# Jiang-Muyun/PointNet12

Hardware: AMD Instinct MI355X
Metric: points/sec fwd+bwd, PointNet2 SemSeg B=16x4096 pts (higher is better)
Workload: dtype f32 (wide-layer products: exact bf16x3 operand splits, 6 bf16 MFMAs per fp32 product, fp32 accumulate)

## Files before the change

### pointnet12_amd/csrc/mlp_res.hip

```cpp
#include "mlp_host.h"
#include "split_bf16.h"

namespace {

constexpr int RES_BM = 64;

struct ResPlan {
    signed char dx_rb[8], dx_cj[8];
    signed char dw_cj[8], dw_q0[8], dw_q1[8];
};

inline bool make_res_plan(int CI_T, ResPlan *out) {
    ResPlan p;
    int load[8], next_q[4] = {0, 0, 0, 0};
    for (int w = 0; w < 8; ++w) { p.dx_rb[w] = p.dx_cj[w] = -1; p.dw_cj[w] = 0; p.dw_q0[w] = p.dw_q1[w] = 0; load[w] = 0; }
    if (CI_T < 1 || CI_T > 4) return false;
    for (int i = 0; i < 2 * CI_T; ++i) { p.dx_rb[i] = (signed char)(i & 1); p.dx_cj[i] = (signed char)(i >> 1); load[i] = 2; }
    const int target = CI_T > 2 ? CI_T : 2;
    for (int pass = 0; pass < 2; ++pass)
        for (int w = 7; w >= 0; --w) {
            if ((pass == 0) != (p.dx_rb[w] < 0) || p.dw_q0[w] != p.dw_q1[w]) continue;
            int cj = -1;
            for (int c = 0; c < CI_T; ++c)
                if (next_q[c] < 4 && (cj < 0 || next_q[c] < next_q[cj])) cj = c;
// ... 612 lines not shown
                            frags(e0, pb, f0);
                            if (two) {
                                frags(e1, pb, f1);
#pragma unroll
                                for (int q = 0; q < 6; ++q) {
                                    accw[DXW ? 0 : j] = __builtin_amdgcn_mfma_f32_32x32x16_bf16(f0[PA[q]].v, f0[PB[q]].v, accw[DXW ? 0 : j], 0, 0, 0);
                                    accw[DXW || j + 1 >= TW ? 0 : j + 1] = __builtin_amdgcn_mfma_f32_32x32x16_bf16(f1[PA[q]].v, f1[PB[q]].v, accw[DXW || j + 1 >= TW ? 0 : j + 1], 0, 0, 0);
                                }
                            } else {
#pragma unroll
                                for (int q = 0; q < 6; ++q)
                                    accw[DXW ? 0 : j] = __builtin_amdgcn_mfma_f32_32x32x16_bf16(f0[PA[q]].v, f0[PB[q]].v, accw[DXW ? 0 : j], 0, 0, 0);
                            }
                        }
                    }
                }
                RSTAMP(3)
            } else {
                f32x16 acc, acc2;
#pragma unroll
                for (int r = 0; r < 16; ++r) { acc[r] = 0.f; acc2[r] = 0.f; }
#pragma unroll
                for (int kb = 0; kb < KBX; ++kb) {
                    const unsigned o = tr_img_off(l31, 2 * kb + lh);
                    SplitFrag ah, am, al;
                    ah.q = *reinterpret_cast<const uint4 *>(ia + o);
                    am.q = *reinterpret_cast<const uint4 *>(ia + o + PANEL);
                    al.q = *reinterpret_cast<const uint4 *>(ia + o + 2 * PANEL);
                    acc = __builtin_amdgcn_mfma_f32_32x32x16_bf16(al.v, wh[DXW ? kb : 0].v, acc, 0, 0, 0);
                    f32x16 &d = DX2 ? acc2 : acc;
                    SplitFrag wlo;
                    if (WL_LDS) wlo.q = wl_lds[kb * 64]; else wlo = wl[DXW && !WL_LDS ? kb : 0];
                    d = __builtin_amdgcn_mfma_f32_32x32x16_bf16(ah.v, wlo.v, d, 0, 0, 0);
                    acc = __builtin_amdgcn_mfma_f32_32x32x16_bf16(am.v, wm[DXW ? kb : 0].v, acc, 0, 0, 0);
                    d = __builtin_amdgcn_mfma_f32_32x32x16_bf16(am.v, wh[DXW ? kb : 0].v, d, 0, 0, 0);
                    acc = __builtin_amdgcn_mfma_f32_32x32x16_bf16(ah.v, wm[DXW ? kb : 0].v, acc, 0, 0, 0);
                    d = __builtin_amdgcn_mfma_f32_32x32x16_bf16(ah.v, wh[DXW ? kb : 0].v, d, 0, 0, 0);
                }
#ifdef PN2_STAMP
                { float a0_ = acc[0] + acc2[0]; asm volatile("" : "+v"(a0_)); }
#endif
                RSTAMP(3)
                const float *yq = Yps + buf * (BP * LDP) + (4 * lh) * LDP + ecol;
                float yv[16];
                if (MASKED) {
#pragma unroll
                    for (int r = 0; r < 16; ++r) yv[r] = yq[((r & 3) + 8 * (r >> 2)) * LDP];
                }
                float *xb = dX + ((size_t)chunk * BP + 4 * lh) * (unsigned)ldxo;
                unsigned offx = (unsigned)ecol;
                asm volatile("" : "+v"(offx));
                float s0 = 0.f, s1 = 0.f;
                const float *x0q = x0s + buf * (BP * 12) + (4 * lh) * 12;
                const unsigned sgn = (unsigned)(chunk & 1) << 31;
#pragma unroll
                for (int r = 0; r < 16; ++r) {
                    float dz = __uint_as_float(__float_as_uint(DX2 ? acc[r] + acc2[r] : acc[r]) ^ sgn);
                    if (MASKED) {
                        const float y = yv[r];
                        dz = bn_act(y, emu, esc, ebe) > 0.f ? dz : 0.f;
                        s0 += dz;
                        s1 = __builtin_fmaf(dz, (y - emu) * eis, s1);
                    }
                    if (FUSE0) {
                        const float4 *xr = reinterpret_cast<const float4 *>(x0q + ((r & 3) + 8 * (r >> 2)) * 12);
                        const float4 a0 = xr[0], a1 = xr[1], a2 = xr[2];
                        g0[0] = __builtin_fmaf(dz, a0.x, g0[0]); g0[FUSE0 ? 1 : 0] = __builtin_fmaf(dz, a0.y, g0[FUSE0 ? 1 : 0]);
                        g0[FUSE0 ? 2 : 0] = __builtin_fmaf(dz, a0.z, g0[FUSE0 ? 2 : 0]); g0[FUSE0 ? 3 : 0] = __builtin_fmaf(dz, a0.w, g0[FUSE0 ? 3 : 0]);
                        g0[FUSE0 ? 4 : 0] = __builtin_fmaf(dz, a1.x, g0[FUSE0 ? 4 : 0]); g0[FUSE0 ? 5 : 0] = __builtin_fmaf(dz, a1.y, g0[FUSE0 ? 5 : 0]);
                        g0[FUSE0 ? 6 : 0] = __builtin_fmaf(dz, a1.z, g0[FUSE0 ? 6 : 0]); g0[FUSE0 ? 7 : 0] = __builtin_fmaf(dz, a1.w, g0[FUSE0 ? 7 : 0]);
                        g0[FUSE0 ? 8 : 0] = __builtin_fmaf(dz, a2.x, g0[FUSE0 ? 8 : 0]); g0[FUSE0 ? 9 : 0] = __builtin_fmaf(dz, a2.y, g0[FUSE0 ? 9 : 0]);
                        g0[FUSE0 ? 10 : 0] = __builtin_fmaf(dz, a2.z, g0[FUSE0 ? 10 : 0]); g0[FUSE0 ? 11 : 0] = __builtin_fmaf(dz, a2.w, g0[FUSE0 ? 11 : 0]);
                    } else {
#if defined(PN2_EXP_NOSTORE)
                        if (dz == 1.2345e-33f) xb[offx] = dz;
#elif defined(PN2_EXP_PLAINSTORE)
                        xb[offx] = dz;
#else
                        PN2_STREAM_STORE(dz, xb + offx);
#endif
                    }
                    offx += ((r & 3) == 3 ? 5u : 1u) * (unsigned)ldxo;
                }
                if (MASKED) { st0 += (double)s0; st1 += (double)s1; }
                RSTAMP(4)
            }
            chunk += G;
            buf ^= 1;
        };
        while (chunk < chunks) {
            iter(D2 ? raw1 : raw0);
            if (chunk >= chunks) break;
            iter(raw0);
        }
        RSTAMP_FLUSH(wave)
        RABS(wave, 2)
        if (!DXW) {
#pragma unroll
            for (int j = 0; j < TW; ++j) {
                const int e = (wave - CI_T) + j * NDW;
                if (e < NTILE) {
                    const int mb = e / CI_T, nb = e - mb * CI_T;
#pragma unroll
                    for (int r = 0; r < 16; ++r)
                        atomicAdd(dW + (int64_t)(mb * 32 + acc_row(r, lh)) * lddw + nb * 32 + l31, accw[DXW ? 0 : j][r]);
                }
            }
        } else if (MASKED && red_p != nullptr) {
            st0 += __shfl_xor(st0, 32, 64);
            st1 += __shfl_xor(st1, 32, 64);
            if (lh == 0) {
                double *rep = red_p + (size_t)(blockIdx.x % PN2_STAT_REPLICAS) * 2 * Ci;
                atomicAdd(rep + ecol, st0);
                atomicAdd(rep + Ci + ecol, st1);
            }
        }
        if (DXW && FUSE0) {
#pragma unroll
            for (int j = 0; j < (DXW && FUSE0 ? 12 : 1); ++j) g0[j] += __shfl_xor(g0[j], 32, 64);
            if (lh == 0) {
                float *pr = part0 + ((size_t)(blockIdx.x % PN2_CF_REPL) * Ci + ecol) * 16;
#pragma unroll
                for (int j = 0; j < (DXW && FUSE0 ? 12 : 1); ++j) atomicAdd(pr + j, g0[j]);
            }
        }
    };
    if (has_dx) run(pn2_true{}); else run(pn2_false{});
    RABS(wave, 3)
}

template <int CO_T, int CI_T, bool POOLED, bool MASKED, bool FUSE0 = false>
int launch_split_bwd_res(ResDy dy, const float *Yp, int ldp, const float *aff_p, const float *W, int ldw, int64_t tiles, float *dX, int ldxo,
                         double *red_p, float *dW, int lddw, hipStream_t s, const float *X0 = nullptr, int ld0 = 0, float *part0 = nullptr) {
    constexpr int Co = 32 * CO_T, Ci = 32 * CI_T;
    constexpr size_t lds = 2 * 6 * (size_t)(32 * 256) + sizeof(float) * (2 * 32 * (Ci + 4) + 8 * Co + 6 * Ci + (FUSE0 ? 2 * 32 * 12 : 0)) +
                           (CO_T == 4 && CI_T < 4 ? (size_t)CI_T * (Co / 16) * 1024 : 0);
    static_assert(lds <= 160 * 1024, "LDS");
    if (!aligned16(dy.Y) || !aligned16(Yp)) return PN2_EUNSUPPORTED;
    auto kern = split_bwd_res_kernel<CO_T, CI_T, POOLED, MASKED, FUSE0>;
    static Pn2PerDevice raised;
    if (pn2_raise_dynamic_lds(reinterpret_cast<const void *>(kern), raised) != PN2_OK) return PN2_ELAUNCH;
    const int64_t chunks = tiles * (RES_BM / 32), cap = pn2_num_cus();
    PN2_NOTE_KERNEL(kern);
    hipLaunchKernelGGL(kern, dim3((unsigned)(chunks < cap ? chunks : cap)), dim3(512), lds, s, dy, Yp, ldp, aff_p, W, ldw, chunks, dX, ldxo,
                       red_p, dW, lddw, X0, ld0, part0);
    return pn2_launch_status();
}

template <int CO_T, int CI_T>
__global__ __launch_bounds__(512, 1) void split_bwd_cf_kernel(const float *dZp, const int32_t *arg, int ldo, int kshift, const float *W2 ,
                                                              const float *Yp, int ldp, const float *aff_p, int64_t chunks, float *dX, int ldxo, double *red_p,
                                                              float *slab) {
    constexpr int Co = 32 * CO_T, Ci = 32 * CI_T, BP = 32, QD = Co / 4, QP = Ci / 4, LDP = Ci + 4;
    constexpr int PANEL = BP * 256, BUF = 6 * PANEL;
    constexpr int KBX = Co / 16, KBM = Ci / 16, KBT = KBX + KBM;
    constexpr int NS = 8 - CI_T - 1, NTS = 64 * NS;
    constexpr int NGT = CI_T * (CI_T + 1) / 2, LDT = Co + Ci + 4;
    static_assert(NS >= CO_T, "one staging wave per D column");
    constexpr int RPP = NTS / QD, IT_D = (BP + RPP - 1) / RPP, IT_P = (BP * QP + NTS - 1) / NTS;
    static_assert(NTS % QD == 0, "one channel quad of D per staging thread");
    unsigned char *lds_b = reinterpret_cast<unsigned char *>(res_lds);
    float *Yps = res_lds + (2 * BUF) / 4;
    float *xtab = Yps + 2 * BP * LDP;
    const int t = threadIdx.x, lane = t & 63, wave = __builtin_amdgcn_readfirstlane(t >> 6), l31 = lane & 31, lh = lane >> 5;
    const int G = gridDim.x;
    RABS(wave, 0)
    for (int i = t; i < 3 * Ci; i += 512) { const float v = aff_p[i]; xtab[i] = v; xtab[3 * Ci + i] = i < Ci ? v : -v; }

    const bool has_dx = wave < CI_T, is_gram = wave == CI_T;
    const int ecol = (has_dx ? wave : 0) * 32 + l31;
    const int ts = wave <= CI_T ? 0 : t - 64 * (CI_T + 1);
    struct Raw { float4 z; int4 a; float4 p[IT_P]; };
    Raw raw;
    auto p_item = [&](int i, int &row, int &q) { const int idx = (NTS * (i + 1) > BP * QP) ? min(ts + NTS * i, BP * QP - 1) : ts + NTS * i; row = idx / QP; q = idx - row * QP; };
    auto fetch = [&](int64_t chunk) {
        const unsigned m0 = (unsigned)(chunk < chunks ? chunk : chunks - 1) * BP;
        const unsigned o = (m0 >> kshift) * (unsigned)ldo + 4u * (unsigned)(ts % QD);
        raw.z = ld4(dZp + o);
        raw.a = ld4i(arg + o);
#pragma unroll
        for (int i = 0; i < IT_P; ++i) {
            int row, q;
            p_item(i, row, q);
            raw.p[i] = ld4(Yp + ((m0 + (unsigned)row) * (unsigned)ldp + 4u * (unsigned)q));
        }
    };
    auto store_split = [&](unsigned char *img, int row, int q, const float4 v) {
        unsigned h0, m0, l0, h1, m1, l1;
        split2(v.x, v.y, h0, m0, l0);
        split2(v.z, v.w, h1, m1, l1);
        const unsigned o = tr_img_off(row, q >> 1) + 8u * (unsigned)(q & 1);
        *reinterpret_cast<uint2 *>(img + o) = make_uint2(h0, h1);
        *reinterpret_cast<uint2 *>(img + o + PANEL) = make_uint2(m0, m1);
        *reinterpret_cast<uint2 *>(img + o + 2 * PANEL) = make_uint2(l0, l1);
    };
    auto stage = [&](int64_t chunk, int buf) {
        unsigned char *ia = lds_b + buf * BUF, *ib = ia + 3 * PANEL;
        float *yp = Yps + buf * (BP * LDP);
        const unsigned m0 = (unsigned)(chunk < chunks ? chunk : chunks - 1) * BP;
        const int kbase = (int)(m0 & ((1u << kshift) - 1u));
        const int par = (int)(chunk & 1);
        const float *xt = xtab + par * (3 * Ci);
        const float lim = par ? -INFINITY : INFINITY;
        {
            unsigned h0, m0_, l0, h1, m1, l1;
            split2(raw.z.x, raw.z.y, h0, m0_, l0);
            split2(raw.z.z, raw.z.w, h1, m1, l1);
            const unsigned sm2 = par ? 0x80008000u : 0u;
            h0 ^= sm2; m0_ ^= sm2; l0 ^= sm2; h1 ^= sm2; m1 ^= sm2; l1 ^= sm2;
            const int q = ts % QD, r0 = ts / QD;
            const int4 a = raw.a;
#pragma unroll
            for (int i = 0; i < IT_D; ++i) {
                const int row = (RPP * (i + 1) > BP) ? min(r0 + RPP * i, BP - 1) : r0 + RPP * i;
                const int k = kbase + row;
                const unsigned k0 = (a.x == k ? 0x0000ffffu : 0u) | (a.y == k ? 0xffff0000u : 0u);
                const unsigned k1 = (a.z == k ? 0x0000ffffu : 0u) | (a.w == k ? 0xffff0000u : 0u);
                const unsigned o = tr_img_off(row, q >> 1) + 8u * (unsigned)(q & 1);
                *reinterpret_cast<uint2 *>(ia + o) = make_uint2(h0 & k0, h1 & k1);
                *reinterpret_cast<uint2 *>(ia + o + PANEL) = make_uint2(m0_ & k0, m1 & k1);
                *reinterpret_cast<uint2 *>(ia + o + 2 * PANEL) = make_uint2(l0 & k0, l1 & k1);
            }
        }
#pragma unroll
        for (int i = 0; i < IT_P; ++i) {
            int row, q;
            p_item(i, row, q);
            float4 x = raw.p[i];
            *reinterpret_cast<float4 *>(&yp[row * LDP + 4 * q]) = x;
            const float4 mu = *reinterpret_cast<const float4 *>(&xt[4 * q]), sc = *reinterpret_cast<const float4 *>(&xt[Ci + 4 * q]);
            const float4 be = *reinterpret_cast<const float4 *>(&xt[2 * Ci + 4 * q]);
            x.x = __builtin_amdgcn_fmed3f(bn_act(x.x, mu.x, sc.x, be.x), 0.f, lim); x.y = __builtin_amdgcn_fmed3f(bn_act(x.y, mu.y, sc.y, be.y), 0.f, lim);
            x.z = __builtin_amdgcn_fmed3f(bn_act(x.z, mu.z, sc.z, be.z), 0.f, lim); x.w = __builtin_amdgcn_fmed3f(bn_act(x.w, mu.w, sc.w, be.w), 0.f, lim);
            store_split(ib, row, q, x);
        }
    };
    auto raw_landed = [&]() {
        asm volatile("" : "+v"(raw.z.x), "+v"(raw.z.y), "+v"(raw.z.z), "+v"(raw.z.w));
        asm volatile("" : "+v"(raw.a.x), "+v"(raw.a.y), "+v"(raw.a.z), "+v"(raw.a.w));
#pragma unroll
        for (int i = 0; i < IT_P; ++i) asm volatile("" : "+v"(raw.p[i].x), "+v"(raw.p[i].y), "+v"(raw.p[i].z), "+v"(raw.p[i].w));
    };
    const int g16 = lane >> 4, j16 = lane & 15, tq = j16 >> 2, tp = j16 & 3;
    auto frag_t = [&](const unsigned char *img, int cblk, int pb) {
        const int c0 = (cblk * 32 + 16 * (g16 & 1)) >> 3;
        SplitFrag f;
#pragma unroll
        for (int r2 = 0; r2 < 2; ++r2) {
            const int row = 16 * pb + 8 * (g16 >> 1) + 4 * r2 + tq;
            const unsigned o = tr_img_off(row, c0 + (tp >> 1)) + 8u * (unsigned)(tp & 1);
            const pn2_s16x4 v = __builtin_amdgcn_ds_read_tr16_b64_v4i16(
                reinterpret_cast<__attribute__((address_space(3))) pn2_s16x4 *>((__attribute__((address_space(3))) unsigned char *)(img) + o));
            const uint2 u = __builtin_bit_cast(uint2, v);
            f.u[2 * r2] = u.x; f.u[2 * r2 + 1] = u.y;
        }
        return f;
    };

    if (has_dx) {
        SplitFrag wh[KBT], wm[KBT], wl[KBM];
        uint4 *wl_lds = reinterpret_cast<uint4 *>(xtab + 6 * Ci) + (size_t)wave * KBX * 64 + lane;
        {
            float v[KBT][8];
#pragma unroll
            for (int kb = 0; kb < KBT; ++kb)
#pragma unroll
                for (int e = 0; e < 8; ++e) v[kb][e] = W2[(16 * kb + 8 * lh + e) * Ci + ecol];
#pragma unroll
            for (int kb = 0; kb < KBT; ++kb) {
                SplitFrag lo;
#pragma unroll
                for (int e = 0; e < 4; ++e) split2(v[kb][2 * e], v[kb][2 * e + 1], wh[kb].u[e], wm[kb].u[e], lo.u[e]);
                if (kb < KBX) wl_lds[kb * 64] = lo.q; else wl[kb < KBX ? 0 : kb - KBX] = lo;
            }
        }
        Affine a(aff_p, Ci);
        const float emu = a.mean[ecol], esc = a.scale[ecol], ebe = a.beta[ecol], eis = a.invstd[ecol];
        const float eh = W2[(Co + Ci) * Ci + ecol];
        double st0 = 0.0, st1 = 0.0, st2 = 0.0;
        int64_t chunk = blockIdx.x;
        int buf = 0;
        __syncthreads();
        RABS(wave, 1)
        RSTAMP_DECL
        while (chunk < chunks) {
            __syncthreads();
            RSTAMP(2)
            const unsigned char *ia = lds_b + buf * BUF, *ib = ia + 3 * PANEL;
            f32x16 acc, acc2;
#pragma unroll
            for (int r = 0; r < 16; ++r) { acc[r] = 0.f; acc2[r] = 0.f; }
#ifndef PN2_X_CF_NODXM
#pragma unroll
            for (int kb = 0; kb < KBT; ++kb) {
                const unsigned char *img = kb < KBX ? ia : ib;
                const unsigned o = tr_img_off(l31, 2 * (kb < KBX ? kb : kb - KBX) + lh);
                SplitFrag ah, am, al, wlo;
                ah.q = *reinterpret_cast<const uint4 *>(img + o);
                am.q = *reinterpret_cast<const uint4 *>(img + o + PANEL);
                al.q = *reinterpret_cast<const uint4 *>(img + o + 2 * PANEL);
                if (kb < KBX) wlo.q = wl_lds[kb * 64]; else wlo = wl[kb < KBX ? 0 : kb - KBX];
                acc = __builtin_amdgcn_mfma_f32_32x32x16_bf16(al.v, wh[kb].v, acc, 0, 0, 0);
                acc2 = __builtin_amdgcn_mfma_f32_32x32x16_bf16(ah.v, wlo.v, acc2, 0, 0, 0);
                acc = __builtin_amdgcn_mfma_f32_32x32x16_bf16(am.v, wm[kb].v, acc, 0, 0, 0);
                acc2 = __builtin_amdgcn_mfma_f32_32x32x16_bf16(am.v, wh[kb].v, acc2, 0, 0, 0);
                acc = __builtin_amdgcn_mfma_f32_32x32x16_bf16(ah.v, wm[kb].v, acc, 0, 0, 0);
                acc2 = __builtin_amdgcn_mfma_f32_32x32x16_bf16(ah.v, wh[kb].v, acc2, 0, 0, 0);
            }
#endif
#ifdef PN2_STAMP
            { float a0_ = acc[0] + acc2[0]; asm volatile("" : "+v"(a0_)); }
#endif
            RSTAMP(3)
#ifdef PN2_X_CF_NOEPI
            if (acc[0] == 1.2345e-33f) dX[0] = acc2[1];
            chunk += G; buf ^= 1;
            continue;
#endif
            const float *yq = Yps + buf * (BP * LDP) + (4 * lh) * LDP + ecol;
            float yv[16];
#pragma unroll
            for (int r = 0; r < 16; ++r) yv[r] = yq[((r & 3) + 8 * (r >> 2)) * LDP];
            float *xb = dX + ((size_t)chunk * BP + 4 * lh) * (unsigned)ldxo;
            unsigned offx = (unsigned)ecol;
            asm volatile("" : "+v"(offx));
            float s0 = 0.f, s1 = 0.f, s2 = 0.f;
            const unsigned sgn = (unsigned)(chunk & 1) << 31;
#pragma unroll
            for (int r = 0; r < 16; ++r) {
                const float y = yv[r];
                const float x = bn_act(y, emu, esc, ebe);
                float dz = __uint_as_float(__float_as_uint(acc[r] + acc2[r]) ^ sgn) + eh;
                dz = x > 0.f ? dz : 0.f;
                s0 += dz;
                s1 = __builtin_fmaf(dz, (y - emu) * eis, s1);
                s2 += fmaxf(x, 0.f);
                PN2_STREAM_STORE(dz, xb + offx);
                offx += ((r & 3) == 3 ? 5u : 1u) * (unsigned)ldxo;
            }
            st0 += (double)s0; st1 += (double)s1; st2 += (double)s2;
            RSTAMP(4)
            chunk += G;
            buf ^= 1;
        }
        RSTAMP_FLUSH(wave)
        RABS(wave, 2)
        st0 += __shfl_xor(st0, 32, 64);
        st1 += __shfl_xor(st1, 32, 64);
        st2 += __shfl_xor(st2, 32, 64);
        if (lh == 0) {
            if (red_p != nullptr) {
                double *rep = red_p + (size_t)(blockIdx.x % PN2_STAT_REPLICAS) * 2 * Ci;
                atomicAdd(rep + ecol, st0);
                atomicAdd(rep + Ci + ecol, st1);
            }
            slab[(size_t)blockIdx.x * (Ci * LDT) + (size_t)ecol * LDT + Co + Ci] = (float)st2;
        }
    } else {
        constexpr int PA[6] = {2, 0, 1, 1, 0, 0}, PB[6] = {0, 2, 1, 0, 1, 0};
        auto mm2 = [&](f32x16 &c0, const SplitFrag (&a0)[3], const SplitFrag (&b0)[3], f32x16 &c1, const SplitFrag (&a1)[3], const SplitFrag (&b1)[3]) {
#pragma unroll
            for (int q = 0; q < 6; ++q) {
                c0 = __builtin_amdgcn_mfma_f32_32x32x16_bf16(a0[PA[q]].v, b0[PB[q]].v, c0, 0, 0, 0);
                c1 = __builtin_amdgcn_mfma_f32_32x32x16_bf16(a1[PA[q]].v, b1[PB[q]].v, c1, 0, 0, 0);
            }
        };
        auto mm1 = [&](f32x16 &c0, const SplitFrag (&a0)[3], const SplitFrag (&b0)[3]) {
#pragma unroll
            for (int q = 0; q < 6; ++q) c0 = __builtin_amdgcn_mfma_f32_32x32x16_bf16(a0[PA[q]].v, b0[PB[q]].v, c0, 0, 0, 0);
        };
        auto frag3 = [&](const unsigned char *img, int blk, int pb, SplitFrag (&f)[3]) {
            f[0] = frag_t(img, blk, pb); f[1] = frag_t(img + PANEL, blk, pb); f[2] = frag_t(img + 2 * PANEL, blk, pb);
        };
        float *sl = slab + (size_t)blockIdx.x * (Ci * LDT);
        if (is_gram) {
            f32x16 accg[NGT];
#pragma unroll
            for (int j = 0; j < NGT; ++j)
#pragma unroll
                for (int r = 0; r < 16; ++r) accg[j][r] = 0.f;
            int64_t chunk = blockIdx.x;
            int buf = 0;
            __syncthreads();
            RABS(wave, 1)
            RSTAMP_DECL
            while (chunk < chunks) {
                __syncthreads();
                RSTAMP(2)
#ifndef PN2_X_CF_NOT
                const unsigned char *ib = lds_b + buf * BUF + 3 * PANEL;
#pragma unroll
                for (int pb = 0; pb < BP / 16; ++pb) {
                    SplitFrag fx[CI_T][3];
#pragma unroll
                    for (int i = 0; i < CI_T; ++i) frag3(ib, i, pb, fx[i]);
                    if constexpr (CI_T == 1) {
                        mm1(accg[0], fx[0], fx[0]);
                    } else if constexpr (CI_T == 2) {
                        mm2(accg[0], fx[0], fx[0], accg[1], fx[0], fx[1]);
                        mm1(accg[2], fx[1], fx[1]);
                    } else {
                        static_assert(CI_T <= 3, "Gram tiles");
                        mm2(accg[0], fx[0], fx[0], accg[1], fx[0], fx[1]);
                        mm2(accg[2], fx[1], fx[1], accg[3], fx[0], fx[2]);
                        mm2(accg[4], fx[1], fx[2], accg[5], fx[2], fx[2]);
                    }
                }
#endif
                RSTAMP(3)
                chunk += G;
                buf ^= 1;
            }
            RSTAMP_FLUSH(wave)
            RABS(wave, 2)
#pragma unroll
            for (int j = 0; j < CI_T; ++j)
#pragma unroll
                for (int i = 0; i <= j; ++i) {
                    const f32x16 &acc = accg[j * (j + 1) / 2 + i];
#pragma unroll
                    for (int r = 0; r < 16; ++r) sl[(i * 32 + acc_row(r, lh)) * LDT + Co + j * 32 + l31] = acc[r];
                    if (i != j) {
#pragma unroll
                        for (int r = 0; r < 16; ++r) sl[(j * 32 + l31) * LDT + Co + i * 32 + acc_row(r, lh)] = acc[r];
                    }
                }
        } else {
            f32x16 accw[CI_T];
#pragma unroll
            for (int j = 0; j < CI_T; ++j)
#pragma unroll
                for (int r = 0; r < 16; ++r) accw[j][r] = 0.f;
            const int nb = wave - CI_T - 1 < CO_T ? wave - CI_T - 1 : -1;
            int64_t chunk = blockIdx.x;
            fetch(chunk);
            __syncthreads();
            stage(chunk, 0);
            fetch(chunk + G);
            raw_landed();
            int buf = 0;
            RABS(wave, 1)
            RSTAMP_DECL
            while (chunk < chunks) {
                __syncthreads();
                RSTAMP(2)
#ifndef PN2_X_CF_NOSTAGE
                stage(chunk + G, buf ^ 1);
#endif
                RSTAMP(0)
#ifndef PN2_X_CF_NOFETCH
                fetch(chunk + 2 * (int64_t)G);
#endif
                __builtin_amdgcn_sched_barrier(0);
                RSTAMP(1)
#ifndef PN2_X_CF_NOT
                if (nb >= 0) {
                    const unsigned char *ia = lds_b + buf * BUF, *ib = ia + 3 * PANEL;
#pragma unroll
                    for (int pb = 0; pb < BP / 16; ++pb) {
                        SplitFrag fb[3], fa0[3], fa1[3];
                        frag3(ia, nb, pb, fb);
                        frag3(ib, 0, pb, fa0);
                        if constexpr (CI_T >= 2) {
                            frag3(ib, 1, pb, fa1);
                            mm2(accw[0], fa0, fb, accw[CI_T >= 2 ? 1 : 0], fa1, fb);
                            if constexpr (CI_T == 3) {
                                frag3(ib, 2, pb, fa0);
                                mm1(accw[CI_T == 3 ? 2 : 0], fa0, fb);
                            }
                        } else {
                            mm1(accw[0], fa0, fb);
                        }
                    }
                }
#endif
                RSTAMP(3)
                chunk += G;
                buf ^= 1;
            }
            RSTAMP_FLUSH(wave)
            RABS(wave, 2)
            if (nb >= 0) {
#pragma unroll
                for (int i = 0; i < CI_T; ++i)
#pragma unroll
                    for (int r = 0; r < 16; ++r) sl[(i * 32 + acc_row(r, lh)) * LDT + nb * 32 + l31] = accw[i][r];
            }
        }
    }
    RABS(wave, 3)
}

__global__ __launch_bounds__(128) void cf_prep_kernel(LazyCoef lc, const float *coef, int ldc, const float *__restrict__ W, int ldw,
                                                      const float *__restrict__ bias, int Co, int Ci, float *__restrict__ W2) {
    __shared__ double fac[256];
    lazy_coef_prologue(lc);
    const float *c0 = coef, *q1 = coef + ldc, *q0 = coef + 2 * ldc, *mean = coef + 3 * ldc;
    const int r = blockIdx.x;
    if (r < Co) {
        for (int i = threadIdx.x; i < Ci; i += 128) W2[r * Ci + i] = c0[r] * W[(int64_t)r * ldw + i];
        return;
    }
    const int j = r - Co;
    for (int c = threadIdx.x; c < Co; c += 128)
        fac[c] = j == Ci ? ((double)q1[c] * ((double)bias[c] - (double)mean[c]) + (double)q0[c]) : (double)W[(int64_t)c * ldw + j] * (double)q1[c];
    __syncthreads();
    for (int i = threadIdx.x; i < Ci; i += 128) {
        double s0 = 0.0, s1 = 0.0, s2 = 0.0, s3 = 0.0;
#pragma unroll 4
        for (int c = 0; c < Co; c += 4) {
            s0 += fac[c] * (double)W[(int64_t)c * ldw + i];
            s1 += fac[c + 1] * (double)W[(int64_t)(c + 1) * ldw + i];
            s2 += fac[c + 2] * (double)W[(int64_t)(c + 2) * ldw + i];
            s3 += fac[c + 3] * (double)W[(int64_t)(c + 3) * ldw + i];
        }
        W2[r * Ci + i] = (float)((s0 + s1) + (s2 + s3));
    }
}

__global__ __launch_bounds__(256) void cf_finish_kernel(const float *__restrict__ slab, int nslab, int Co, int Ci, const float *coef, int ldc,
                                                        const float *__restrict__ W, int ldw, const float *__restrict__ bias,
                                                        float *__restrict__ dW, int lddw) {
    extern __shared__ double cf_row[];
    const int i = blockIdx.x, LDT = Co + Ci + 4, NQ = LDT / 4;
    const int q = threadIdx.x & 63, sg = threadIdx.x >> 6;
    double a0 = 0.0, a1 = 0.0, a2 = 0.0, a3 = 0.0;
    if (q < NQ) {
        const float *p = slab + (size_t)i * LDT + 4 * q;
        const size_t ss = (size_t)Ci * LDT;
        int w = sg;
        for (; w + 28 < nslab; w += 32) {
            float4 v[8];
#pragma unroll
            for (int e = 0; e < 8; ++e) v[e] = ld4(p + (size_t)(w + 4 * e) * ss);
#pragma unroll
            for (int e = 0; e < 8; ++e) { a0 += (double)v[e].x; a1 += (double)v[e].y; a2 += (double)v[e].z; a3 += (double)v[e].w; }
        }
        for (; w < nslab; w += 4) {
            const float4 v = ld4(p + (size_t)w * ss);
            a0 += (double)v.x; a1 += (double)v.y; a2 += (double)v.z; a3 += (double)v.w;
        }
        double *d = cf_row + sg * LDT + 4 * q;
        d[0] = a0; d[1] = a1; d[2] = a2; d[3] = a3;
    }
    __syncthreads();
    for (int n = threadIdx.x; n < LDT; n += 256) cf_row[n] = (cf_row[n] + cf_row[LDT + n]) + (cf_row[2 * LDT + n] + cf_row[3 * LDT + n]);
    __syncthreads();
    const float *c0 = coef, *q1 = coef + ldc, *q0 = coef + 2 * ldc, *mean = coef + 3 * ldc;
    const double sx = cf_row[Co + Ci];
    for (int c = threadIdx.x; c < Co; c += 256) {
        double dot = 0.0;
        for (int j = 0; j < Ci; ++j) dot += (double)W[(int64_t)c * ldw + j] * cf_row[Co + j];
        const double g = (double)c0[c] * cf_row[c] + (double)q1[c] * (dot + ((double)bias[c] - (double)mean[c]) * sx) + (double)q0[c] * sx;
        dW[(int64_t)c * lddw + i] += (float)g;
    }
}

template <int CO_T, int CI_T>
int launch_split_bwd_cf(const float *dZp, const int32_t *arg, int ldo, int kshift, const float *coef, LazyCoef lc, const float *W, int ldw,
                        const float *bias, const float *Yp, int ldp, const float *aff_p, int64_t P, float *dX, int ldxo, double *red_p,
                        float *dW, int lddw, float *scratch, hipStream_t s) {
    constexpr int Co = 32 * CO_T, Ci = 32 * CI_T, LDT = Co + Ci + 4;
    constexpr size_t lds = 2 * 6 * (size_t)(32 * 256) + sizeof(float) * (2 * 32 * (Ci + 4) + 6 * Ci) + (size_t)CI_T * (Co / 16) * 1024;
    static_assert(lds <= 160 * 1024, "LDS");
    auto kern = split_bwd_cf_kernel<CO_T, CI_T>;
    static Pn2PerDevice raised;
    if (pn2_raise_dynamic_lds(reinterpret_cast<const void *>(kern), raised) != PN2_OK) return PN2_ELAUNCH;
    float *W2 = scratch, *slab = scratch + (((Co + Ci + 1) * Ci + 63) & ~63);
    const int64_t chunks = P / 32, cap = pn2_num_cus() < 256 ? pn2_num_cus() : 256;
    const int grid = (int)(chunks < cap ? chunks : cap);
    hipLaunchKernelGGL(cf_prep_kernel, dim3(Co + Ci + 1), dim3(128), 0, s, lc, coef, round4(Co), W, ldw, bias, Co, Ci, W2);
    PN2_NOTE_KERNEL(kern);
    hipLaunchKernelGGL(kern, dim3((unsigned)grid), dim3(512), lds, s, dZp, arg, ldo, kshift, W2, Yp, ldp, aff_p, chunks, dX, ldxo, red_p, slab);
    hipLaunchKernelGGL(cf_finish_kernel, dim3(Ci), dim3(256), sizeof(double) * 4 * LDT, s, slab, grid, Co, Ci, coef, round4(Co), W, ldw, bias,
                       dW, lddw);
    return pn2_launch_status();
}

#define PN2_RES_CASE(CO, CI, POOL, MASKED)                                                                                \
    if (Co == CO && Ci == CI)                                                                                              \
        return launch_bwd_res<CO / 32, CI / 32, POOL, MASKED>(dy, Yp, ldp, aff_p, W, ldw, tiles, dX, ldxo, red_p, dW, lddw, s);

int dispatch_bwd_res(int Kpool, bool masked, int Co, int Ci, ResDy dy, const float *Yp, int ldp, const float *aff_p, const float *W,
                     int ldw, int64_t tiles, float *dX, int ldxo, double *red_p, float *dW, int lddw, hipStream_t s) {
    if (pn2_opt(PN2_OPT_SPLIT) && pn2_opt(PN2_OPT_SPLIT_RES)) {
#define PN2_SPLIT_RES_CASE(CO, CI, POOLED, MASKED)                                                                        \
        if (Co == CO && Ci == CI) {                                                                                        \
            const int rc = launch_split_bwd_res<CO / 32, CI / 32, POOLED, MASKED>(dy, Yp, ldp, aff_p, W, ldw, tiles, dX, ldxo, red_p, dW, lddw, s); \
            if (rc != PN2_EUNSUPPORTED) return rc;                                                                         \
        }
        const bool all = pn2_opt(PN2_OPT_SPLIT_RES) >= 2;
        if (Kpool == 0 && masked) {
            if (all) { PN2_SPLIT_RES_CASE(32, 32, false, true) }
            PN2_SPLIT_RES_CASE(64, 64, false, true) PN2_SPLIT_RES_CASE(96, 64, false, true)
            if (tiles >= pn2_opt(PN2_OPT_SPLIT_RES_MIN_TILES_128)) { PN2_SPLIT_RES_CASE(128, 128, false, true) }
        } else if (Kpool == 0) {
            if (tiles >= pn2_opt(PN2_OPT_SPLIT_RES_MIN_TILES_128)) { PN2_SPLIT_RES_CASE(128, 128, false, false) }
        } else if (masked && Kpool % 32 == 0) {
            if (all) { PN2_SPLIT_RES_CASE(64, 32, true, true) }
            PN2_SPLIT_RES_CASE(128, 64, true, true) PN2_SPLIT_RES_CASE(128, 96, true, true)
        }
#undef PN2_SPLIT_RES_CASE
    }
    if (Kpool == 0 && masked) {
        PN2_RES_CASE(32, 32, 0, true) PN2_RES_CASE(64, 64, 0, true) PN2_RES_CASE(96, 64, 0, true)
        if (tiles >= 4096) { PN2_RES_CASE(128, 128, 0, true) }
    } else if (Kpool == 0) {
        if (tiles >= 4096) { PN2_RES_CASE(128, 128, 0, false) }
    } else if (masked && Kpool % 64 == 0) {
        PN2_RES_CASE(128, 64, 1, true) PN2_RES_CASE(128, 96, 1, true)
    } else if (masked && Kpool == 32) {
        PN2_RES_CASE(64, 32, 2, true) PN2_RES_CASE(128, 64, 2, true)
    }
    return PN2_EUNSUPPORTED;
}

struct ResPool {
    float2 *rec;
    const float *gamma;
    int ldp, U;
    LazyBn lz;
};

template <int K_T, int N_T, bool ACT, int POOL>
__global__ __launch_bounds__(512, 2) void fwd_res_kernel(const float *__restrict__ X, int ldx, const float *aff ,
                                                         const float *__restrict__ W, int ldw, const float *__restrict__ bias,
                                                         float *__restrict__ Y, int ldy, int64_t slabs, double *__restrict__ stats,
                                                         ResPool pool) {
    constexpr int K = 32 * K_T, N = 32 * N_T, LDA = K + 4, QK = K / 4, IT = 32 * QK / 64;
    const int NW = blockDim.x >> 6;
    float *Ws = res_lds;
    float *atab = Ws + N * LDA;
    const int t = threadIdx.x, lane = t & 63, wave = __builtin_amdgcn_readfirstlane(t >> 6), l31 = lane & 31, lh = lane >> 5;
    float *Ab = atab + 3 * K + wave * (32 * LDA);
    RABS(wave, 0)

    lazy_bn_prologue(pool.lz);
    for (int i = t; i < N * QK; i += blockDim.x) {
        const int n = i / QK, q = i - n * QK;
        const float *src = W + (int64_t)n * ldw + 4 * q;
        float4 v;
        if ((ldw & 3) == 0 && (reinterpret_cast<uintptr_t>(W) & 15) == 0) v = ld4(src);
        else v = make_float4(src[0], src[1], src[2], src[3]);
        *reinterpret_cast<float4 *>(&Ws[n * LDA + 4 * q]) = v;
    }
    if (ACT)
        for (int i = t; i < 3 * K; i += blockDim.x) atab[i] = aff[i];
    float bj[N_T];
#pragma unroll
    for (int j = 0; j < N_T; ++j) bj[j] = bias[32 * j + l31];

    constexpr bool OFFS_LIVE = POOL == 0;
    unsigned ox[OFFS_LIVE ? IT : 1], ol[OFFS_LIVE ? IT : 1];
    int lane_op = lane;
    auto off_x = [&](int i) { const int idx = lane_op + 64 * i, row = idx / QK, q = idx - row * QK; return (unsigned)row * (unsigned)ldx + 4u * q; };
    auto off_l = [&](int i) { const int idx = lane_op + 64 * i, row = idx / QK, q = idx - row * QK; return (unsigned)(row * LDA + 4 * q); };
    if (OFFS_LIVE) {
#pragma unroll
        for (int i = 0; i < IT; ++i) { ox[OFFS_LIVE ? i : 0] = off_x(i); ol[OFFS_LIVE ? i : 0] = off_l(i); }
    }
    const int64_t stride = (int64_t)gridDim.x * NW;
    float4 rx[IT];
    auto fetch = [&](int64_t slab) {
        const float *xb = X + (slab < slabs ? slab : slabs - 1) * (int64_t)(32 * ldx);
#pragma unroll
        for (int i = 0; i < IT; ++i) rx[i] = ld4(xb + (OFFS_LIVE ? ox[OFFS_LIVE ? i : 0] : off_x(i)));
    };
    const int U = POOL ? pool.U : 1;
    int64_t unit = (int64_t)blockIdx.x * NW + wave;
    int sub = 0;
    int64_t slab = unit * U;
    fetch(slab);
    double st[N_T][2];
#pragma unroll
    for (int j = 0; j < N_T; ++j) st[j][0] = st[j][1] = 0.0;
    float vmx[POOL ? N_T : 1];
    int kmx[POOL ? N_T : 1], sgn[POOL ? N_T : 1];
    if (POOL) {
#pragma unroll
        for (int j = 0; j < N_T; ++j) sgn[POOL ? j : 0] = pool.gamma[32 * j + l31] < 0.f ? (int)0x80000000 : 0;
    }
    __syncthreads();
    constexpr bool AT_HOIST = ACT && 64 % QK == 0 && !(K_T == 4 && N_T == 4);
    float4 hmu, hsc, hbe;
    if (AT_HOIST) {
        const int q4 = 4 * (lane % QK);
        hmu = *reinterpret_cast<const float4 *>(&atab[q4]);
        hsc = *reinterpret_cast<const float4 *>(&atab[K + q4]);
        hbe = *reinterpret_cast<const float4 *>(&atab[2 * K + q4]);
    }

    RSTAMP_DECL
    RABS(wave, 1)
    while (slab < slabs) {
        RSTAMP(4)
        if (!OFFS_LIVE) asm volatile("" : "+v"(lane_op));
        int64_t next_unit = unit;
        int next_sub = sub + 1;
        if (next_sub == U) { next_sub = 0; next_unit += stride; }
        const int64_t next_slab = next_unit * U + next_sub;
#pragma unroll
        for (int i = 0; i < IT; ++i) {
            float4 x = rx[i];
            const unsigned oli = OFFS_LIVE ? ol[OFFS_LIVE ? i : 0] : off_l(i);
            if (ACT) {
                const int q4 = AT_HOIST ? 0 : (int)(oli % (unsigned)LDA);
                const float4 mu = AT_HOIST ? hmu : *reinterpret_cast<const float4 *>(&atab[q4]);
                const float4 sc = AT_HOIST ? hsc : *reinterpret_cast<const float4 *>(&atab[K + q4]);
                const float4 be = AT_HOIST ? hbe : *reinterpret_cast<const float4 *>(&atab[2 * K + q4]);
                x.x = fmaxf(bn_act(x.x, mu.x, sc.x, be.x), 0.f);
                x.y = fmaxf(bn_act(x.y, mu.y, sc.y, be.y), 0.f);
                x.z = fmaxf(bn_act(x.z, mu.z, sc.z, be.z), 0.f);
                x.w = fmaxf(bn_act(x.w, mu.w, sc.w, be.w), 0.f);
            }
            *reinterpret_cast<float4 *>(&Ab[oli]) = x;
        }
// ... 361 lines not shown
```

Before: 13.62 million.

## Exploit sparse max-pool gradient in CF backward via scatter lists instead of dense MFMA

The backward kernel used to expand the pooled gradient into a dense masked bf16x3 panel and feed it through MFMAs for both dX and the dW cross term. It now builds a per-wave list of the few nonzero (channel, row) entries with ballot and mbcnt, and scatter-adds dz*W into an LDS accumulator with workgroup-scope atomics. The dW cross term is accumulated by owner threads with scalar FMAs over the selected rows, and the freed waves take over some Gram tiles. This removes the D-panel splitting and its MFMAs, but it adds LDS atomics, a full fp32 W copy in LDS, and the kernel is now restricted to CO_T=4 with CI_T of 2 or 3.

```diff
diff --git a/pointnet12_amd/csrc/mlp_res.hip b/pointnet12_amd/csrc/mlp_res.hip
--- a/pointnet12_amd/csrc/mlp_res.hip
+++ b/pointnet12_amd/csrc/mlp_res.hip
@@ -788,26 +788,37 @@
                                                               const float *Yp, int ldp, const float *aff_p, int64_t chunks, float *dX, int ldxo, double *red_p,
                                                               float *slab) {
     constexpr int Co = 32 * CO_T, Ci = 32 * CI_T, BP = 32, QD = Co / 4, QP = Ci / 4, LDP = Ci + 4;
-    constexpr int PANEL = BP * 256, BUF = 6 * PANEL;
-    constexpr int KBX = Co / 16, KBM = Ci / 16, KBT = KBX + KBM;
+    constexpr int PANEL = BP * 256, BUF = 3 * PANEL;
+    constexpr int KBM = Ci / 16;
     constexpr int NS = 8 - CI_T - 1, NTS = 64 * NS;
     constexpr int NGT = CI_T * (CI_T + 1) / 2, LDT = Co + Ci + 4;
-    static_assert(NS >= CO_T, "one staging wave per D column");
-    constexpr int RPP = NTS / QD, IT_D = (BP + RPP - 1) / RPP, IT_P = (BP * QP + NTS - 1) / NTS;
-    static_assert(NTS % QD == 0, "one channel quad of D per staging thread");
+    constexpr int NGM = CI_T == 3 ? 4 : 2;
+    constexpr int TDR = Ci / 8;
+    constexpr int NB = (Ci + 63) / 64;
+    static_assert(CO_T == 4 && (CI_T == 2 || CI_T == 3), "the deal of Gram tiles and the 8-bit channel of a list entry");
+    static_assert(QD == 32 && NS >= 4 && NGT - NGM <= NS - NB && TDR % 4 == 0, "a quad per lane of a half wave; owners, builders");
+    constexpr int IT_P = (BP * QP + NTS - 1) / NTS;
     unsigned char *lds_b = reinterpret_cast<unsigned char *>(res_lds);
     float *Yps = res_lds + (2 * BUF) / 4;
     float *xtab = Yps + 2 * BP * LDP;
+    float *Wf = xtab + 6 * Ci;
+    float *Es = Wf + Co * Ci;
+    uint2 *lst = reinterpret_cast<uint2 *>(Es + 2 * BP * LDP);
     const int t = threadIdx.x, lane = t & 63, wave = __builtin_amdgcn_readfirstlane(t >> 6), l31 = lane & 31, lh = lane >> 5;
     const int G = gridDim.x;
     RABS(wave, 0)
     for (int i = t; i < 3 * Ci; i += 512) { const float v = aff_p[i]; xtab[i] = v; xtab[3 * Ci + i] = i < Ci ? v : -v; }
+    for (int i = t; i < Co * Ci / 4; i += 512) reinterpret_cast<float4 *>(Wf)[i] = ld4(W2 + 4 * i);
+    for (int i = t; i < 2 * BP * LDP / 4; i += 512) reinterpret_cast<float4 *>(Es)[i] = make_float4(0.f, 0.f, 0.f, 0.f);
 
     const bool has_dx = wave < CI_T, is_gram = wave == CI_T;
     const int ecol = (has_dx ? wave : 0) * 32 + l31;
     const int ts = wave <= CI_T ? 0 : t - 64 * (CI_T + 1);
+    const int eb = wave - (8 - NB);
     struct Raw { float4 z; int4 a; float4 p[IT_P]; };
     Raw raw;
+    float4 cz = make_float4(0.f, 0.f, 0.f, 0.f);
+    uint4 ck = make_uint4(~0u, ~0u, ~0u, ~0u);
     auto p_item = [&](int i, int &row, int &q) { const int idx = (NTS * (i + 1) > BP * QP) ? min(ts + NTS * i, BP * QP - 1) : ts + NTS * i; row = idx / QP; q = idx - row * QP; };
     auto fetch = [&](int64_t chunk) {
         const unsigned m0 = (unsigned)(chunk < chunks ? chunk : chunks - 1) * BP;
@@ -831,32 +842,53 @@
         *reinterpret_cast<uint2 *>(img + o + 2 * PANEL) = make_uint2(l0, l1);
     };
     auto stage = [&](int64_t chunk, int buf) {
-        unsigned char *ia = lds_b + buf * BUF, *ib = ia + 3 * PANEL;
+        unsigned char *ib = lds_b + buf * BUF;
         float *yp = Yps + buf * (BP * LDP);
         const unsigned m0 = (unsigned)(chunk < chunks ? chunk : chunks - 1) * BP;
-        const int kbase = (int)(m0 & ((1u << kshift) - 1u));
+        const unsigned kbase = m0 & ((1u << kshift) - 1u);
         const int par = (int)(chunk & 1);
         const float *xt = xtab + par * (3 * Ci);
         const float lim = par ? -INFINITY : INFINITY;
-        {
-            unsigned h0, m0_, l0, h1, m1, l1;
-            split2(raw.z.x, raw.z.y, h0, m0_, l0);
-            split2(raw.z.z, raw.z.w, h1, m1, l1);
-            const unsigned sm2 = par ? 0x80008000u : 0u;
-            h0 ^= sm2; m0_ ^= sm2; l0 ^= sm2; h1 ^= sm2; m1 ^= sm2; l1 ^= sm2;
-            const int q = ts % QD, r0 = ts / QD;
-            const int4 a = raw.a;
-#pragma unroll
-            for (int i = 0; i < IT_D; ++i) {
-                const int row = (RPP * (i + 1) > BP) ? min(r0 + RPP * i, BP - 1) : r0 + RPP * i;
-                const int k = kbase + row;
-                const unsigned k0 = (a.x == k ? 0x0000ffffu : 0u) | (a.y == k ? 0xffff0000u : 0u);
-                const unsigned k1 = (a.z == k ? 0x0000ffffu : 0u) | (a.w == k ? 0xffff0000u : 0u);
-                const unsigned o = tr_img_off(row, q >> 1) + 8u * (unsigned)(q & 1);
-                *reinterpret_cast<uint2 *>(ia + o) = make_uint2(h0 & k0, h1 & k1);
-                *reinterpret_cast<uint2 *>(ia + o + PANEL) = make_uint2(m0_ & k0, m1 & k1);
-                *reinterpret_cast<uint2 *>(ia + o + 2 * PANEL) = make_uint2(l0 & k0, l1 & k1);
-            }
+        cz = raw.z;
+        ck = make_uint4((unsigned)raw.a.x - kbase, (unsigned)raw.a.y - kbase, (unsigned)raw.a.z - kbase, (unsigned)raw.a.w - kbase);
+        if (eb >= 0) {
+            const float z0 = lh ? cz.z : cz.x, z1 = lh ? cz.w : cz.y;
+            const unsigned k0 = lh ? ck.z : ck.x, k1 = lh ? ck.w : ck.y, c0 = 4u * (unsigned)l31 + 2u * (unsigned)lh;
+            const bool h0 = k0 < (unsigned)BP, h1 = k1 < (unsigned)BP;
+            const unsigned long long b0 = __ballot(h0), b1 = __ballot(h1);
+            const int n0 = __popcll(b0), nnz = n0 + __popcll(b1);
+            const int p0 = (int)__builtin_amdgcn_mbcnt_hi((unsigned)(b0 >> 32), __builtin_amdgcn_mbcnt_lo((unsigned)b0, 0u));
+            const int p1 = n0 + (int)__builtin_amdgcn_mbcnt_hi((unsigned)(b1 >> 32), __builtin_amdgcn_mbcnt_lo((unsigned)b1, 0u));
+            uint2 *lw = lst + eb * Co;
+            if (h0) lw[p0] = make_uint2(c0 | (k0 << 8), __float_as_uint(z0));
+            if (h1) lw[p1] = make_uint2((c0 + 1u) | (k1 << 8), __float_as_uint(z1));
+            __builtin_amdgcn_wave_barrier();
+            uint2 e0 = lw[lane], e1 = lw[lane + 64];
+            if (lane >= nnz) e0 = make_uint2(0u, 0u);
+            if (lane + 64 >= nnz) e1 = make_uint2(0u, 0u);
+            __builtin_amdgcn_wave_barrier();
+            float *ecolp = Es + buf * (BP * LDP) + 64 * eb + lane;
+            const float *wcol = Wf + 64 * eb + lane;
+            const bool has_col = 64 * eb + lane < Ci;
+            auto add4 = [&](const uint2 e, int n) {
+                unsigned key[4];
+                float dzv[4], w[4];
+#pragma unroll
+                for (int u = 0; u < 4; ++u) {
+                    key[u] = (unsigned)__builtin_amdgcn_readlane((int)e.x, n + u);
+                    dzv[u] = __uint_as_float((unsigned)__builtin_amdgcn_readlane((int)e.y, n + u));
+                }
+                if (has_col) {
+#pragma unroll
+                    for (int u = 0; u < 4; ++u) w[u] = wcol[(key[u] & 0xffu) * Ci];
+#pragma unroll
+                    for (int u = 0; u < 4; ++u)
+                        (void)__hip_atomic_fetch_add(ecolp + (key[u] >> 8) * LDP, dzv[u] * w[u], __ATOMIC_RELAXED, __HIP_MEMORY_SCOPE_WORKGROUP);
+                }
+            };
+            const int nr = (nnz + 3) & ~3;
+            for (int n = 0; n < (nr < 64 ? nr : 64); n += 4) add4(e0, n);
+            for (int n = 64; n < nr; n += 4) add4(e1, n - 64);
         }
 #pragma unroll
         for (int i = 0; i < IT_P; ++i) {
@@ -894,21 +926,17 @@
     };
 
     if (has_dx) {
-        SplitFrag wh[KBT], wm[KBT], wl[KBM];
-        uint4 *wl_lds = reinterpret_cast<uint4 *>(xtab + 6 * Ci) + (size_t)wave * KBX * 64 + lane;
+        SplitFrag wh[KBM], wm[KBM], wl[KBM];
         {
-            float v[KBT][8];
-#pragma unroll
-            for (int kb = 0; kb < KBT; ++kb)
-#pragma unroll
-                for (int e = 0; e < 8; ++e) v[kb][e] = W2[(16 * kb + 8 * lh + e) * Ci + ecol];
-#pragma unroll
-            for (int kb = 0; kb < KBT; ++kb) {
-                SplitFrag lo;
-#pragma unroll
-                for (int e = 0; e < 4; ++e) split2(v[kb][2 * e], v[kb][2 * e + 1], wh[kb].u[e], wm[kb].u[e], lo.u[e]);
-                if (kb < KBX) wl_lds[kb * 64] = lo.q; else wl[kb < KBX ? 0 : kb - KBX] = lo;
-            }
+            float v[KBM][8];
+#pragma unroll
+            for (int kb = 0; kb < KBM; ++kb)
+#pragma unroll
+                for (int e = 0; e < 8; ++e) v[kb][e] = W2[(Co + 16 * kb + 8 * lh + e) * Ci + ecol];
+#pragma unroll
+            for (int kb = 0; kb < KBM; ++kb)
+#pragma unroll
+                for (int e = 0; e < 4; ++e) split2(v[kb][2 * e], v[kb][2 * e + 1], wh[kb].u[e], wm[kb].u[e], wl[kb].u[e]);
         }
         Affine a(aff_p, Ci);
         const float emu = a.mean[ecol], esc = a.scale[ecol], ebe = a.beta[ecol], eis = a.invstd[ecol];
@@ -922,22 +950,20 @@
         while (chunk < chunks) {
             __syncthreads();
             RSTAMP(2)
-            const unsigned char *ia = lds_b + buf * BUF, *ib = ia + 3 * PANEL;
+            const unsigned char *ib = lds_b + buf * BUF;
             f32x16 acc, acc2;
 #pragma unroll
             for (int r = 0; r < 16; ++r) { acc[r] = 0.f; acc2[r] = 0.f; }
 #ifndef PN2_X_CF_NODXM
 #pragma unroll
-            for (int kb = 0; kb < KBT; ++kb) {
-                const unsigned char *img = kb < KBX ? ia : ib;
-                const unsigned o = tr_img_off(l31, 2 * (kb < KBX ? kb : kb - KBX) + lh);
-                SplitFrag ah, am, al, wlo;
-                ah.q = *reinterpret_cast<const uint4 *>(img + o);
-                am.q = *reinterpret_cast<const uint4 *>(img + o + PANEL);
-                al.q = *reinterpret_cast<const uint4 *>(img + o + 2 * PANEL);
-                if (kb < KBX) wlo.q = wl_lds[kb * 64]; else wlo = wl[kb < KBX ? 0 : kb - KBX];
+            for (int kb = 0; kb < KBM; ++kb) {
+                const unsigned o = tr_img_off(l31, 2 * kb + lh);
+                SplitFrag ah, am, al;
+                ah.q = *reinterpret_cast<const uint4 *>(ib + o);
+                am.q = *reinterpret_cast<const uint4 *>(ib + o + PANEL);
+                al.q = *reinterpret_cast<const uint4 *>(ib + o + 2 * PANEL);
                 acc = __builtin_amdgcn_mfma_f32_32x32x16_bf16(al.v, wh[kb].v, acc, 0, 0, 0);
-                acc2 = __builtin_amdgcn_mfma_f32_32x32x16_bf16(ah.v, wlo.v, acc2, 0, 0, 0);
+                acc2 = __builtin_amdgcn_mfma_f32_32x32x16_bf16(ah.v, wl[kb].v, acc2, 0, 0, 0);
                 acc = __builtin_amdgcn_mfma_f32_32x32x16_bf16(am.v, wm[kb].v, acc, 0, 0, 0);
                 acc2 = __builtin_amdgcn_mfma_f32_32x32x16_bf16(am.v, wh[kb].v, acc2, 0, 0, 0);
                 acc = __builtin_amdgcn_mfma_f32_32x32x16_bf16(ah.v, wm[kb].v, acc, 0, 0, 0);
@@ -957,6 +983,12 @@
             float yv[16];
 #pragma unroll
             for (int r = 0; r < 16; ++r) yv[r] = yq[((r & 3) + 8 * (r >> 2)) * LDP];
+            float *eq = Es + buf * (BP * LDP) + (4 * lh) * LDP + ecol;
+            float ev[16];
+#pragma unroll
+            for (int r = 0; r < 16; ++r) ev[r] = eq[((r & 3) + 8 * (r >> 2)) * LDP];
+#pragma unroll
+            for (int r = 0; r < 16; ++r) eq[((r & 3) + 8 * (r >> 2)) * LDP] = 0.f;
             float *xb = dX + ((size_t)chunk * BP + 4 * lh) * (unsigned)ldxo;
             unsigned offx = (unsigned)ecol;
             asm volatile("" : "+v"(offx));
@@ -966,7 +998,7 @@
             for (int r = 0; r < 16; ++r) {
                 const float y = yv[r];
                 const float x = bn_act(y, emu, esc, ebe);
-                float dz = __uint_as_float(__float_as_uint(acc[r] + acc2[r]) ^ sgn) + eh;
+                float dz = (__uint_as_float(__float_as_uint(acc[r] + acc2[r]) ^ sgn) + ev[r]) + eh;
                 dz = x > 0.f ? dz : 0.f;
                 s0 += dz;
                 s1 = __builtin_fmaf(dz, (y - emu) * eis, s1);
@@ -1001,18 +1033,22 @@
                 c1 = __builtin_amdgcn_mfma_f32_32x32x16_bf16(a1[PA[q]].v, b1[PB[q]].v, c1, 0, 0, 0);
             }
         };
-        auto mm1 = [&](f32x16 &c0, const SplitFrag (&a0)[3], const SplitFrag (&b0)[3]) {
-#pragma unroll
-            for (int q = 0; q < 6; ++q) c0 = __builtin_amdgcn_mfma_f32_32x32x16_bf16(a0[PA[q]].v, b0[PB[q]].v, c0, 0, 0, 0);
-        };
         auto frag3 = [&](const unsigned char *img, int blk, int pb, SplitFrag (&f)[3]) {
             f[0] = frag_t(img, blk, pb); f[1] = frag_t(img + PANEL, blk, pb); f[2] = frag_t(img + 2 * PANEL, blk, pb);
         };
         float *sl = slab + (size_t)blockIdx.x * (Ci * LDT);
+        auto flush_gram = [&](const f32x16 &acc, int i, int j) {
+#pragma unroll
+            for (int r = 0; r < 16; ++r) sl[(i * 32 + acc_row(r, lh)) * LDT + Co + j * 32 + l31] = acc[r];
+            if (i != j) {
+#pragma unroll
+                for (int r = 0; r < 16; ++r) sl[(j * 32 + l31) * LDT + Co + i * 32 + acc_row(r, lh)] = acc[r];
+            }
+        };
         if (is_gram) {
-            f32x16 accg[NGT];
-#pragma unroll
-            for (int j = 0; j < NGT; ++j)
+            f32x16 accg[NGM];
+#pragma unroll
+            for (int j = 0; j < NGM; ++j)
 #pragma unroll
                 for (int r = 0; r < 16; ++r) accg[j][r] = 0.f;
             int64_t chunk = blockIdx.x;
@@ -1024,23 +1060,14 @@
                 __syncthreads();
                 RSTAMP(2)
 #ifndef PN2_X_CF_NOT
-                const unsigned char *ib = lds_b + buf * BUF + 3 * PANEL;
+                const unsigned char *ib = lds_b + buf * BUF;
 #pragma unroll
                 for (int pb = 0; pb < BP / 16; ++pb) {
                     SplitFrag fx[CI_T][3];
 #pragma unroll
                     for (int i = 0; i < CI_T; ++i) frag3(ib, i, pb, fx[i]);
-                    if constexpr (CI_T == 1) {
-                        mm1(accg[0], fx[0], fx[0]);
-                    } else if constexpr (CI_T == 2) {
-                        mm2(accg[0], fx[0], fx[0], accg[1], fx[0], fx[1]);
-                        mm1(accg[2], fx[1], fx[1]);
-                    } else {
-                        static_assert(CI_T <= 3, "Gram tiles");
-                        mm2(accg[0], fx[0], fx[0], accg[1], fx[0], fx[1]);
-                        mm2(accg[2], fx[1], fx[1], accg[3], fx[0], fx[2]);
-                        mm2(accg[4], fx[1], fx[2], accg[5], fx[2], fx[2]);
-                    }
+                    mm2(accg[0], fx[0], fx[0], accg[1], fx[0], fx[1]);
+                    if constexpr (CI_T == 3) mm2(accg[2], fx[1], fx[1], accg[NGM - 1], fx[0], fx[CI_T - 1]);
                 }
 #endif
                 RSTAMP(3)
@@ -1052,25 +1079,30 @@
 #pragma unroll
             for (int j = 0; j < CI_T; ++j)
 #pragma unroll
-                for (int i = 0; i <= j; ++i) {
-                    const f32x16 &acc = accg[j * (j + 1) / 2 + i];
-#pragma unroll
-                    for (int r = 0; r < 16; ++r) sl[(i * 32 + acc_row(r, lh)) * LDT + Co + j * 32 + l31] = acc[r];
-                    if (i != j) {
-#pragma unroll
-                        for (int r = 0; r < 16; ++r) sl[(j * 32 + l31) * LDT + Co + i * 32 + acc_row(r, lh)] = acc[r];
-                    }
-                }
+                for (int i = 0; i <= j; ++i)
+                    if (j * (j + 1) / 2 + i < NGM) flush_gram(accg[j * (j + 1) / 2 + i < NGM ? j * (j + 1) / 2 + i : 0], i, j);
         } else {
-            f32x16 accw[CI_T];
-#pragma unroll
-            for (int j = 0; j < CI_T; ++j)
-#pragma unroll
-                for (int r = 0; r < 16; ++r) accw[j][r] = 0.f;
-            const int nb = wave - CI_T - 1 < CO_T ? wave - CI_T - 1 : -1;
+            const int sw = wave - CI_T - 1, gi = sw < NGT - NGM ? CI_T - (NGT - NGM) + sw : -1;
+            const int q = ts % QD, r0 = ts / QD;
+            const bool owner = r0 < 8;
+            f32x16 accx[2];
+#pragma unroll
+            for (int j = 0; j < 2; ++j)
+#pragma unroll
+                for (int r = 0; r < 16; ++r) accx[j][r] = 0.f;
+            float td[4][TDR], tmu[TDR], tsc[TDR], tbe[TDR];
+#pragma unroll
+            for (int e = 0; e < 4; ++e)
+#pragma unroll
+                for (int i = 0; i < TDR; ++i) td[e][i] = 0.f;
             int64_t chunk = blockIdx.x;
             fetch(chunk);
             __syncthreads();
+#pragma unroll
+            for (int i = 0; i < TDR; ++i) {
+                const int ch = TDR * (r0 & 7) + i;
+                tmu[i] = xtab[ch]; tsc[i] = xtab[Ci + ch]; tbe[i] = xtab[2 * Ci + ch];
+            }
             stage(chunk, 0);
             fetch(chunk + G);
             raw_landed();
@@ -1080,6 +1112,31 @@
             while (chunk < chunks) {
                 __syncthreads();
                 RSTAMP(2)
+#ifndef PN2_X_CF_NOT
+                if (owner) {
+                    const float zc[4] = {cz.x, cz.y, cz.z, cz.w};
+                    const unsigned kc[4] = {ck.x, ck.y, ck.z, ck.w};
+#pragma unroll
+                    for (int e = 0; e < 4; ++e) {
+                        if (kc[e] < (unsigned)BP) {
+                            const float *yr = Yps + buf * (BP * LDP) + kc[e] * LDP + TDR * r0;
+                            float z = zc[e];
+                            PN2_OPAQUE1(z);
+#pragma unroll
+                            for (int i4 = 0; i4 < TDR / 4; ++i4) {
+                                float4 y = *reinterpret_cast<const float4 *>(yr + 4 * i4);
+                                PN2_OPAQUE4(y.x, y.y, y.z, y.w);
+                                const float yy[4] = {y.x, y.y, y.z, y.w};
+#pragma unroll
+                                for (int u = 0; u < 4; ++u) {
+                                    const int i = 4 * i4 + u;
+                                    td[e][i] = __builtin_fmaf(z, fmaxf(bn_act(yy[u], tmu[i], tsc[i], tbe[i]), 0.f), td[e][i]);
+                                }
+                            }
+                        }
+                    }
+                }
+#endif
 #ifndef PN2_X_CF_NOSTAGE
                 stage(chunk + G, buf ^ 1);
 #endif
@@ -1090,24 +1147,14 @@
                 __builtin_amdgcn_sched_barrier(0);
                 RSTAMP(1)
 #ifndef PN2_X_CF_NOT
-                if (nb >= 0) {
-                    const unsigned char *ia = lds_b + buf * BUF, *ib = ia + 3 * PANEL;
-#pragma unroll
-                    for (int pb = 0; pb < BP / 16; ++pb) {
-                        SplitFrag fb[3], fa0[3], fa1[3];
-                        frag3(ia, nb, pb, fb);
-                        frag3(ib, 0, pb, fa0);
-                        if constexpr (CI_T >= 2) {
-                            frag3(ib, 1, pb, fa1);
-                            mm2(accw[0], fa0, fb, accw[CI_T >= 2 ? 1 : 0], fa1, fb);
-                            if constexpr (CI_T == 3) {
-                                frag3(ib, 2, pb, fa0);
-                                mm1(accw[CI_T == 3 ? 2 : 0], fa0, fb);
-                            }
-                        } else {
-                            mm1(accw[0], fa0, fb);
-                        }
-                    }
+                if (gi >= 0) {
+                    const unsigned char *ib = lds_b + buf * BUF;
+                    SplitFrag fa0[3], fb0[3], fa1[3], fb1[3];
+                    frag3(ib, gi, 0, fa0);
+                    frag3(ib, CI_T - 1, 0, fb0);
+                    frag3(ib, gi, 1, fa1);
+                    frag3(ib, CI_T - 1, 1, fb1);
+                    mm2(accx[0], fa0, fb0, accx[1], fa1, fb1);
                 }
 #endif
                 RSTAMP(3)
@@ -1116,11 +1163,15 @@
             }
             RSTAMP_FLUSH(wave)
             RABS(wave, 2)
-            if (nb >= 0) {
-#pragma unroll
-                for (int i = 0; i < CI_T; ++i)
-#pragma unroll
-                    for (int r = 0; r < 16; ++r) sl[(i * 32 + acc_row(r, lh)) * LDT + nb * 32 + l31] = accw[i][r];
+            if (gi >= 0) {
+#pragma unroll
+                for (int r = 0; r < 16; ++r) accx[0][r] += accx[1][r];
+                flush_gram(accx[0], gi, CI_T - 1);
+            }
+            if (owner) {
+#pragma unroll
+                for (int i = 0; i < TDR; ++i)
+                    *reinterpret_cast<float4 *>(&sl[(TDR * r0 + i) * LDT + 4 * q]) = make_float4(td[0][i], td[1][i], td[2][i], td[3][i]);
             }
         }
     }
@@ -1197,7 +1248,7 @@
                         const float *bias, const float *Yp, int ldp, const float *aff_p, int64_t P, float *dX, int ldxo, double *red_p,
                         float *dW, int lddw, float *scratch, hipStream_t s) {
     constexpr int Co = 32 * CO_T, Ci = 32 * CI_T, LDT = Co + Ci + 4;
-    constexpr size_t lds = 2 * 6 * (size_t)(32 * 256) + sizeof(float) * (2 * 32 * (Ci + 4) + 6 * Ci) + (size_t)CI_T * (Co / 16) * 1024;
+    constexpr size_t lds = 2 * 3 * (size_t)(32 * 256) + sizeof(float) * (2 * 2 * 32 * (Ci + 4) + 6 * Ci + Co * Ci) + (size_t)((Ci + 63) / 64) * Co * 8;
     static_assert(lds <= 160 * 1024, "LDS");
     auto kern = split_bwd_cf_kernel<CO_T, CI_T>;
     static Pn2PerDevice raised;
```

After: 10.66 million. 0.783x the previous value.
